# risc0/zeth

Measured on AMD Instinct MI355X. Metric: segments/sec, higher is better.
Workload: dtype u32

## Files before the change

### zeth_amd/build.py

```python
from __future__ import annotations

import hashlib
import os
import subprocess
import sys
from concurrent.futures import ThreadPoolExecutor

HERE = os.path.dirname(os.path.abspath(__file__))
CSRC = os.path.join(HERE, "csrc")
ROOT = os.path.dirname(HERE)
VARIANT = os.environ.get("ZKH_BUILD_VARIANT", "")
LIB = os.path.join(ROOT, ".variants", f"libzkhal_{VARIANT}.so") if VARIANT else os.path.join(HERE, "libzkhal_mi355x.so")
OBJ_DIR = os.path.join(ROOT, ".variants", f"_obj_{VARIANT}") if VARIANT else os.path.join(HERE, "csrc", "_obj")
SOURCES = ["hal.hip", "ntt.hip", "hash.hip", "poly.hip", "circuit.hip", "prover.hip", "verifier.hip", "session.hip", "recursion.hip", "topology.hip", "preflight.hip", "rec_builder.hip", "arguments.hip", "accumulate.hip", "multiplicities.hip", "sort.hip", "columns.hip", "links.hip", "image.hip", "check_rows.hip", "bus.hip"]
HIPCC = os.environ.get("HIPCC", "/opt/rocm/bin/hipcc")
FLAGS = ["--offload-arch=gfx950", "-O3", "-std=c++17", "-fPIC", "-Wno-comment", "-Wno-unused-result"] + os.environ.get("ZKH_BUILD_FLAGS", "").split()
EXTRA_FLAGS = {"hash.hip": ["-mllvm", "-enable-misched=0"], "accumulate.hip": ["-mllvm", "-pragma-unroll-threshold=200000"]}


def _extra(src: str) -> list:
    if src.startswith("eval_check_gen"):
        from .circuits import codegen
        return EXTRA_FLAGS.get(src, []) + codegen.KERNEL_FLAGS
    return EXTRA_FLAGS.get(src, [])


def _deps_digest(src: str) -> str:
    h = hashlib.sha256()
    files = [os.path.join(CSRC, src)]
    files += sorted(os.path.join(CSRC, f) for f in os.listdir(CSRC) if f.endswith(".h"))
    files += [os.path.join(ROOT, "include", f) for f in sorted(os.listdir(os.path.join(ROOT, "include")))]
    for f in files:
        with open(f, "rb") as fh:
            h.update(fh.read())
    h.update(" ".join(FLAGS + _extra(src)).encode())
    return h.hexdigest()


def _compile(src: str, force: bool) -> str:
    obj = os.path.join(OBJ_DIR, src.replace(".hip", ".o"))
    stamp = obj + ".sha"
    digest = _deps_digest(src)
    if not force and os.path.exists(obj) and os.path.exists(stamp) and open(stamp).read() == digest:
        return obj
    if src.startswith("eval_check_gen"):
        from .circuits import bounds
        with open(os.path.join(CSRC, src)) as fh:
            violations, _ = bounds.check_source(fh.read(), src)
        if violations:
            raise RuntimeError(f"{src}: the generated kernels are NOT within bounds (circuits/codegen.py's lazy-arithmetic accounting is wrong); "
                               f"not compiled:\n" + "\n".join(violations[:5]))
    cmd = [HIPCC, *FLAGS, *_extra(src), "-c", os.path.join(CSRC, src), "-o", obj]
    r = subprocess.run(cmd, capture_output=True, text=True)
    if r.returncode != 0:
        raise RuntimeError(f"hipcc failed for {src}:\n{r.stderr[-4000:]}")
    with open(stamp, "w") as fh:
        fh.write(digest)
    return obj


def generate_eval_check() -> list:
    from .circuits import codegen
    return codegen.write_generated(CSRC)


def generate_circuit_descs() -> str:
    import numpy as np
    from .circuits import codegen
    lines = ["// GENERATED by zeth_amd/build.py generate_circuit_descs — do not edit.  The shipped circuit descriptions (circuits/*.py) as data.",
             "#include <cstddef>", "#include <cstdint>", '#include "common.h"', ""]
    names = []
    for name, desc in codegen.shipped().items():
        d = np.asarray(desc, dtype=np.uint32)
        names.append((name, d.size))
        lines.append(f"static const uint32_t desc_{name}[{d.size}] = {{")
        for i in range(0, d.size, 16):
            lines.append("    " + ", ".join(f"0x{int(w):x}" for w in d[i:i + 16]) + ",")
        lines.append("};")
    lines += ["", "namespace {", "struct Shipped { const char* name; const uint32_t* words; size_t n; };", "const Shipped k_shipped[] = {"]
    lines += [f'    {{"{n}", desc_{n}, {sz}}},' for n, sz in names]
    lines += ["};", "}  // namespace", "",
              'extern "C" size_t zkh_shipped_circuit_count() { return sizeof(k_shipped) / sizeof(k_shipped[0]); }',
              'extern "C" const char* zkh_shipped_circuit_name(size_t i) { return i < zkh_shipped_circuit_count() ? k_shipped[i].name : nullptr; }',
              'extern "C" const char* zkh_shipped_circuit_desc(const char* name, const uint32_t** words, size_t* n_words) {',
              '    ZKH_REQUIRE(name && words && n_words, "shipped_circuit_desc: null argument");',
              "    for (const Shipped& s : k_shipped)",
              "        if (strcmp(s.name, name) == 0) { *words = s.words; *n_words = s.n; return nullptr; }",
              '    return zkh::make_err("shipped_circuit_desc: no circuit named %s is built into this library", name);',
              "}", ""]
    src = "\n".join(lines)
    path = os.path.join(CSRC, "circuit_descs_gen.hip")
    try:
        with open(path) as fh:
            if fh.read() == src:
                return "circuit_descs_gen.hip"
    except FileNotFoundError:
        pass
    with open(path, "w") as fh:
        fh.write(src)
    return "circuit_descs_gen.hip"


def build_examples() -> str:
    outs = []
    for name in ("seal_segments", "prove_session", "verify_receipts"):
        src = os.path.join(ROOT, "examples", name + ".cpp")
        out = os.path.join(ROOT, "examples", name)
        outs.append(out)
        deps = [src, os.path.join(ROOT, "include", "zkhal.h"), LIB]
        if os.path.exists(out) and all(os.path.getmtime(out) >= os.path.getmtime(d) for d in deps):
            continue
        cmd = ["g++", "-O2", "-std=c++17", "-Wall", "-I", os.path.join(ROOT, "include"), src, "-o", out, "-L", HERE,
               "-lzkhal_mi355x", "-Wl,-rpath,$ORIGIN/../zeth_amd", "-Wl,-rpath-link,/opt/rocm/lib", "-lpthread"]
        r = subprocess.run(cmd, capture_output=True, text=True)
        if r.returncode != 0:
            raise RuntimeError(f"g++ failed for examples/{name}.cpp:\n{r.stderr[-4000:]}")
    return outs[0]


def build_oracle() -> None:
    subprocess.check_call(["make", "-s", "-C", os.path.join(ROOT, "oracle")])


def build(force: bool = False, verbose: bool = False) -> str:
    os.makedirs(OBJ_DIR, exist_ok=True)
    sources = SOURCES + generate_eval_check() + [generate_circuit_descs()]
    wanted = {s.replace(".hip", ".o") for s in sources}
    for f in os.listdir(OBJ_DIR):
        if f.startswith("eval_check_gen") and f.endswith(".o") and f not in wanted:
            os.remove(os.path.join(OBJ_DIR, f))
    with ThreadPoolExecutor(max_workers=min(os.cpu_count() or 4, len(sources))) as ex:
        objs = list(ex.map(lambda s: _compile(s, force), sources))
    newest = max(os.path.getmtime(o) for o in objs)
    if force or not os.path.exists(LIB) or os.path.getmtime(LIB) < newest:
        cmd = [HIPCC, "--offload-arch=gfx950", "-shared", "-fPIC", *objs, "-o", LIB]
        r = subprocess.run(cmd, capture_output=True, text=True)
        if r.returncode != 0:
            raise RuntimeError(f"link failed:\n{r.stderr[-4000:]}")
    if not VARIANT:
        build_examples()
    if verbose:
        print("built", LIB)
    return LIB


def ensure_built(oracle: bool = False, verbose: bool = False) -> str:
    import fcntl
    stamp = os.path.join(OBJ_DIR, ".tree.sha")
    oracle_built = lambda: any(f.endswith(".so") for f in os.listdir(os.path.join(ROOT, "oracle")))
    try:
        with open(stamp) as fh:
            if os.path.exists(LIB) and fh.read() == _tree_digest() and (not oracle or os.environ.get("ZKH_NO_ORACLE_BUILD") or oracle_built()):
                return LIB
    except OSError:
        pass
    os.makedirs(OBJ_DIR, exist_ok=True)
    with open(os.path.join(OBJ_DIR, ".lock"), "w") as lock:
        fcntl.flock(lock, fcntl.LOCK_EX)
        try:
            digest = _tree_digest()
            current = os.path.exists(LIB) and os.path.exists(stamp) and open(stamp).read() == digest
            if not current:
                build(verbose=verbose)
                with open(stamp, "w") as fh:
                    fh.write(digest)
            if oracle and not os.environ.get("ZKH_NO_ORACLE_BUILD") and not (current and oracle_built()):
                build_oracle()
        finally:
            fcntl.flock(lock, fcntl.LOCK_UN)
    return LIB


def record_tree() -> None:
    os.makedirs(OBJ_DIR, exist_ok=True)
    stamp = os.path.join(OBJ_DIR, ".tree.sha")
    with open(stamp + ".tmp", "w") as fh:
        fh.write(_tree_digest())
    os.replace(stamp + ".tmp", stamp)


def _tree_digest() -> str:
    h = hashlib.sha256()
    files = [os.path.join(CSRC, f) for f in sorted(os.listdir(CSRC))
             if (f.endswith(".hip") or f.endswith(".h")) and not f.startswith("eval_check_gen") and f != "circuit_descs_gen.hip"]
    files += [os.path.join(ROOT, "include", f) for f in sorted(os.listdir(os.path.join(ROOT, "include")))]
    files += [os.path.join(HERE, "circuits", f) for f in sorted(os.listdir(os.path.join(HERE, "circuits"))) if f.endswith((".py", ".json"))]
    files += [os.path.abspath(__file__)] + [os.path.join(ROOT, "examples", f) for f in sorted(os.listdir(os.path.join(ROOT, "examples"))) if f.endswith(".cpp")]
    files += [os.path.join(ROOT, "oracle", f) for f in sorted(os.listdir(os.path.join(ROOT, "oracle"))) if f.endswith((".c", ".h")) or f == "Makefile"]
    for f in files:
        with open(f, "rb") as fh:
            h.update(f.encode() + b"\0" + fh.read())
    h.update(" ".join(FLAGS).encode())
# ... 7 lines not shown
```

### zeth_amd/csrc/common.h

```cpp
#pragma once
#include <hip/hip_runtime.h>

#include <atomic>
#include <cstdarg>
#include <cstdio>
#include <cstdlib>
#include <cstring>
#include <map>
#include <string>
#include <vector>

#include "../../include/zkhal.h"
#include "fp.h"
#include "noise.h"

namespace zkh {

inline const char* make_err(const char* fmt, ...) {
    char buf[512];
    va_list ap;
    va_start(ap, fmt);
    vsnprintf(buf, sizeof buf, fmt, ap);
    va_end(ap);
    return strdup(buf);
}
#define ZKH_HIP(expr)                                                                               \
    do {                                                                                            \
        hipError_t _e = (expr);                                                                     \
        if (_e != hipSuccess) return zkh::make_err("%s failed: %s (%s:%d)", #expr, hipGetErrorString(_e), __FILE__, __LINE__); \
    } while (0)
#define ZKH_TRY(expr)                    \
    do {                                 \
        const char* _err = (expr);       \
        if (_err) return _err;           \
    } while (0)
#define ZKH_REQUIRE(cond, ...)                         \
    do {                                               \
        if (!(cond)) return zkh::make_err(__VA_ARGS__); \
    } while (0)

constexpr int ZKH_P2_PTAB = 486;
constexpr int TW_BITS = 12;
constexpr int TW_SIZE = 1 << TW_BITS;
constexpr int TW_HI_BITS = 14;
constexpr int TW_HI_SIZE = 1 << TW_HI_BITS;
constexpr int MAX_LOG_N = TW_BITS + TW_HI_BITS;
constexpr int LDS_TW_LOG = 12;

struct DeviceTables {
    uint32_t* rc;
    uint32_t* diag;
    uint32_t* tw_fwd_lo; uint32_t* tw_fwd_hi;
    uint32_t* tw_rev_lo; uint32_t* tw_rev_hi;
    uint32_t* tile_fwd;  uint32_t* tile_rev;
    uint32_t* layer_fwd; uint32_t* layer_rev;
    uint32_t* layer_fwd_lazy;
    uint32_t* shift_lo;  uint32_t* shift_hi;
};

struct ProfAgg { uint64_t calls = 0; double ms = 0; double bytes = 0; };
struct ProfPending { std::string name; hipEvent_t a, b; double bytes; };

}

struct zkh_alloc_t {
    void* ptr;
    size_t bytes;
    std::atomic<int> refs;
    bool owned;
    zkh_ctx* ctx;
    zkh_alloc_t(void* p, size_t b, int r, bool o, zkh_ctx* c) : ptr(p), bytes(b), refs(r), owned(o), ctx(c) {}
};

struct zkh_buf {
    zkh_alloc_t* a;
    size_t off, len;
    std::atomic<int> refs;
    zkh_buf(zkh_alloc_t* al, size_t o, size_t l, int r) : a(al), off(o), len(l), refs(r) {}
    uint32_t* ptr() const { return (uint32_t*)a->ptr + off; }
};

struct zkh_ctx {
    int device;
    hipStream_t stream;
    zkh::DeviceTables tab;
    uint32_t rou_fwd[28], rou_rev[28];
    uint32_t h_rc[24 * 29], h_diag[zkh::ZKH_P2_PTAB];
    std::multimap<size_t, void*> pool;
    size_t pool_bytes = 0, live_bytes = 0, peak_bytes = 0;
    bool prof = false;
    std::vector<zkh::ProfPending> pending;
    std::map<std::string, zkh::ProfAgg> agg;
    std::vector<hipEvent_t> event_pool;
    uint32_t* pinned = nullptr;
    size_t pinned_words = 0;
    size_t stage_next = 0, stage_used = 0;
    uint32_t* d_fail = nullptr;
    uint32_t* h_fail = nullptr;
    bool fail_armed = false;
    std::map<void*, size_t> host_blocks;
    size_t h2d_bytes = 0;
};

namespace zkh {

const char* pool_alloc(zkh_ctx* c, size_t bytes, void** out);
void pool_free(zkh_ctx* c, void* p, size_t bytes);
const char* new_buf(zkh_ctx* c, size_t n_words, bool zero, zkh_buf** out);
void prof_begin(zkh_ctx* c, const char* name, double bytes);
void prof_end(zkh_ctx* c);
// ... 38 lines not shown
```

### zeth_amd/csrc/hal.hip

```cpp
#include <algorithm>

#include "common.h"

#include <sys/random.h>
#include "poseidon2.h"
#include "ntt_lazy.h"
#include "../../include/zkh_poseidon2_consts.h"

using namespace zkh;

extern "C" void zkh_free_error(const char* e) { free((void*)e); }
#if ZKH_P2_CONSTS_ARE_PLACEHOLDER
extern "C" const char* zkh_version(void) { return "zkhal-mi355x 0.2.0 (gfx950; poseidon2_consts=placeholder)"; }
#elif ZKH_P2_CONSTS_ARE_DERIVED
extern "C" const char* zkh_version(void) { return "zkhal-mi355x 0.2.0 (gfx950; poseidon2_consts=derived)"; }
#else
extern "C" const char* zkh_version(void) { return "zkhal-mi355x 0.2.0 (gfx950; poseidon2_consts=upstream)"; }
#endif

namespace zkh {

const char* pool_alloc(zkh_ctx* c, size_t bytes, void** out) {
    bytes = (bytes + 255) & ~(size_t)255;
    if (bytes == 0) bytes = 256;
// ... 147 lines not shown
        c->rou_rev[k] = fp_inv(w).v;
    }
    Fp wf = Fp::raw(c->rou_fwd[MAX_LOG_N]), wr = Fp::raw(c->rou_rev[MAX_LOG_N]);
    ZKH_TRY(upload(&c->tab.tw_fwd_lo, powers(wf, TW_SIZE)));
    ZKH_TRY(upload(&c->tab.tw_fwd_hi, powers(fp_pow(wf, TW_SIZE), TW_HI_SIZE)));
    ZKH_TRY(upload(&c->tab.tw_rev_lo, powers(wr, TW_SIZE)));
    ZKH_TRY(upload(&c->tab.tw_rev_hi, powers(fp_pow(wr, TW_SIZE), TW_HI_SIZE)));
    ZKH_TRY(upload(&c->tab.tile_fwd, powers(Fp::raw(c->rou_fwd[LDS_TW_LOG]), 1 << (LDS_TW_LOG - 1))));
    ZKH_TRY(upload(&c->tab.tile_rev, powers(Fp::raw(c->rou_rev[LDS_TW_LOG]), 1 << (LDS_TW_LOG - 1))));
    {
        std::vector<uint32_t> lf(1 << LDS_TW_LOG, R1), lr(1 << LDS_TW_LOG, R1);
        for (int j = 1; j <= LDS_TW_LOG; j++) {
            auto pf = powers(Fp::raw(c->rou_fwd[j]), (size_t)1 << (j - 1)), pr = powers(Fp::raw(c->rou_rev[j]), (size_t)1 << (j - 1));
            for (size_t e = 0; e < pf.size(); e++) { lf[((size_t)1 << (j - 1)) + e] = pf[e]; lr[((size_t)1 << (j - 1)) + e] = pr[e]; }
        }
        ZKH_TRY(upload(&c->tab.layer_fwd, lf));
        ZKH_TRY(upload(&c->tab.layer_rev, lr));
        static_assert(LAZY_TAB_LOG == LDS_TW_LOG, "the lazy table covers the per-layer tables");
        std::vector<uint32_t> lz(LAZY_TAB_WORDS);
        lazy_layer_table(lz.data(), lf.data());
        ZKH_TRY(upload(&c->tab.layer_fwd_lazy, lz));
    }
    Fp three = fp_encode(3);
    ZKH_TRY(upload(&c->tab.shift_lo, powers(three, TW_SIZE)));
    ZKH_TRY(upload(&c->tab.shift_hi, powers(fp_pow(three, TW_SIZE), TW_HI_SIZE)));
    ZKH_TRY(upload(&c->tab.rc, std::vector<uint32_t>(24 * 29)));
    ZKH_TRY(upload(&c->tab.diag, std::vector<uint32_t>(ZKH_P2_PTAB)));
    ZKH_TRY(zkh_poseidon2_set_constants(c, ZKH_P2_ROUND_CONSTANTS, ZKH_P2_M_INT_DIAG));
    ZKH_TRY(ntt_device_init(c));
    ZKH_HIP(hipMalloc((void**)&c->d_fail, 8));
    ZKH_HIP(hipMemsetAsync(c->d_fail, 0, 8, c->stream));
    ZKH_HIP(hipHostMalloc((void**)&c->h_fail, 8, hipHostMallocDefault));
    c->h_fail[0] = c->h_fail[1] = 0;
    return nullptr;
}
extern "C" const char* zkh_ctx_trim(zkh_ctx* c) {
    bind_thread(c);
    ZKH_HIP(hipStreamSynchronize(c->stream));
    for (auto& kv : c->pool) (void)hipFree(kv.second);
    c->pool.clear(); c->pool_bytes = 0;
    return nullptr;
}
extern "C" void zkh_ctx_memory(const zkh_ctx* c, size_t* live, size_t* cached, size_t* peak) {
    if (live) *live = c->live_bytes;
    if (cached) *cached = c->pool_bytes;
    if (peak) *peak = c->peak_bytes;
}
extern "C" void zkh_ctx_destroy(zkh_ctx* c) {
    if (!c) return;
    (void)hipSetDevice(c->device);
    (void)hipStreamSynchronize(c->stream);
    for (auto& kv : c->pool) (void)hipFree(kv.second);
    uint32_t* t[] = {c->tab.rc, c->tab.diag, c->tab.tw_fwd_lo, c->tab.tw_fwd_hi, c->tab.tw_rev_lo, c->tab.tw_rev_hi,
                     c->tab.tile_fwd, c->tab.tile_rev, c->tab.shift_lo, c->tab.shift_hi, c->tab.layer_fwd, c->tab.layer_rev, c->tab.layer_fwd_lazy};
    for (auto p : t) (void)hipFree(p);
    for (auto& p : c->pending) { (void)hipEventDestroy(p.a); (void)hipEventDestroy(p.b); }
    for (auto ev : c->event_pool) (void)hipEventDestroy(ev);
    if (c->pinned) (void)hipHostFree(c->pinned);
    if (c->d_fail) (void)hipFree(c->d_fail);
    if (c->h_fail) (void)hipHostFree(c->h_fail);
    for (auto& kv : c->host_blocks) (void)hipHostFree(kv.first);
    (void)hipStreamDestroy(c->stream);
    delete c;
}
static const char* check_device_fail(zkh_ctx* c) {
    if (!c->fail_armed) return nullptr;
    c->fail_armed = false;
    const uint32_t code = c->h_fail[0], detail = c->h_fail[1];
    if (!code) return nullptr;
    (void)hipMemsetAsync(c->d_fail, 0, 8, c->stream);
    switch (code) {
    case 1: return make_err("combos_prepare_regs: register %u has size 0 or more than `cycles` words (found on the device; the call's combos are unchanged)", detail);
    case 2: return make_err("combos_prepare_regs: register %u names a combo beyond combo_count (found on the device; the call's combos are unchanged)", detail);
    case 3: return make_err("combos_prepare_regs: the register sizes add up to %u U coefficients (+ %d of the check polynomial), more than coeff_u holds (found on the device; the call's combos are unchanged)", detail, ZKH_CHECK_SIZE);
    default: return make_err("a kernel reported failure code %u (%u)", code, detail);
    }
}
static const char* sync_checked(zkh_ctx* c) {
    if (c->fail_armed) ZKH_HIP(hipMemcpyAsync(c->h_fail, c->d_fail, 8, hipMemcpyDeviceToHost, c->stream));
    ZKH_HIP(hipStreamSynchronize(c->stream));
    c->stage_used = 0;
    return check_device_fail(c);
}
extern "C" const char* zkh_sync(zkh_ctx* c) {
    bind_thread(c);
    return sync_checked(c);
}
extern "C" void* zkh_ctx_stream(zkh_ctx* c) { return (void*)c->stream; }

extern "C" const char* zkh_alloc(zkh_ctx* c, const char*, size_t n, int zero, zkh_buf** out) {
    return new_buf(c, n, zero != 0, out);
}
namespace zkh {
constexpr size_t STAGE_SLOT_WORDS = 16384, STAGE_SLOTS = 64;
const char* h2d(zkh_ctx* c, uint32_t* dst, const uint32_t* host, size_t n) {
    if (!n) return nullptr;
    bind_thread(c);
    c->h2d_bytes += n * 4;
    if (n <= STAGE_SLOT_WORDS) {
        ZKH_TRY(ensure_pinned(c, STAGE_SLOT_WORDS * STAGE_SLOTS));
        if (c->stage_used == STAGE_SLOTS) ZKH_TRY(sync_checked(c));
        uint32_t* slot = c->pinned + (size_t)c->stage_next * STAGE_SLOT_WORDS;
        memcpy(slot, host, n * 4);
        ZKH_HIP(hipMemcpyAsync(dst, slot, n * 4, hipMemcpyHostToDevice, c->stream));
        c->stage_next = (c->stage_next + 1) % STAGE_SLOTS;
        c->stage_used++;
        return nullptr;
// ... 388 lines not shown
```

### zeth_amd/csrc/ntt.hip

```cpp
#include "common.h"
#include "ntt_lazy.h"

using namespace zkh;

namespace {

constexpr int NTT_THREADS = 256;

struct PassParams {
    const uint32_t* in;
    uint32_t* out;
    size_t in_col_stride;
    size_t out_col_stride;
    uint32_t log_n;
    uint32_t L, R;
    uint32_t log_t;
    uint32_t expand_bits;
    uint32_t first_layer;
    uint32_t twiddle;
    uint32_t scale;
    uint32_t zk_shift;
    const uint32_t* tile_tw;
    const uint32_t* layer_tw;
    const uint32_t* tw_lo;
    const uint32_t* tw_hi;
    const uint32_t* sh_lo;
    const uint32_t* sh_hi;
    uint32_t tiles_per_col;
    uint32_t lazy;
    uint32_t lazy_comp;
    uint32_t shift16[16];
};

template <bool INVERSE>
__global__ __launch_bounds__(NTT_THREADS) void k_ntt_pass(PassParams p) {
    extern __shared__ __attribute__((aligned(16))) uint32_t tile[];
    const uint32_t T = 1u << p.log_t, rows = 1u << p.R, elems = rows << p.log_t;
    const uint32_t tid = threadIdx.x;
    const uint32_t tile_id = xcd_remap(blockIdx.x, p.tiles_per_col);
    const uint32_t col = blockIdx.y;
    const uint32_t ltiles = 1u << (p.L - p.log_t);
    const uint32_t a = tile_id >> (p.L - p.log_t), lt = tile_id & (ltiles - 1);
    const size_t base = ((size_t)a << (p.L + p.R)) + ((size_t)lt << p.log_t);
    const uint32_t l0 = lt << p.log_t;
    const uint32_t* in = p.in + (size_t)col * p.in_col_stride;
    uint32_t* out = p.out + (size_t)col * p.out_col_stride;
    const uint32_t tw_shift = MAX_LOG_N - (p.L + p.R);
    const uint32_t pad_mask = INVERSE ? 0u : (1u << p.expand_bits) - (1u << (p.first_layer - 1));

    for (uint32_t e = tid; e < elems; e += NTT_THREADS) {
        const uint32_t m = e >> p.log_t, t = e & (T - 1);
        const size_t gi = base + ((size_t)m << p.L) + t;
        uint32_t v = (gi & pad_mask) ? 0u : in[gi >> p.expand_bits];
        if (!INVERSE && p.twiddle) {
            const uint32_t r = __brev(m) >> (32 - p.R);
            const uint32_t ex = ((l0 + t) * r) << tw_shift;
            const uint32_t w = mul_mod(p.tw_lo[ex & (TW_SIZE - 1)], p.tw_hi[ex >> TW_BITS]);
            v = mul_mod(v, w);
        }
        tile[e] = v;
    }
    __syncthreads();

    const uint32_t half_elems = elems >> 1;
    if (INVERSE) {
        for (uint32_t j = p.R; j >= 1; j--) {
            const uint32_t hb = j - 1;
            for (uint32_t q = tid; q < half_elems; q += NTT_THREADS) {
                const uint32_t t = q & (T - 1), mm = q >> p.log_t;
                const uint32_t low = mm & ((1u << hb) - 1), m = ((mm >> hb) << j) | low;
                const uint32_t i0 = (m << p.log_t) | t, i1 = i0 + (1u << (hb + p.log_t));
                const uint32_t x = tile[i0], y = tile[i1];
                const uint32_t w = p.tile_tw[low << (LDS_TW_LOG - j)];
                tile[i0] = add_mod(x, y);
                tile[i1] = mul_mod(x - y + P, w);
            }
            __syncthreads();
        }
    } else {
        for (uint32_t j = p.first_layer; j <= p.R; j++) {
            const uint32_t hb = j - 1;
            for (uint32_t q = tid; q < half_elems; q += NTT_THREADS) {
                const uint32_t t = q & (T - 1), mm = q >> p.log_t;
                const uint32_t low = mm & ((1u << hb) - 1), m = ((mm >> hb) << j) | low;
// ... 358 lines not shown
                }
                radix_layers<2, false, true, 1, LAZY>(u, ltab, 0, 0);
#pragma unroll
                for (int k = 0; k < 4; k++) lds[(m0 + k) * TW + t] = u[k];
            }
            __syncthreads();
#pragma unroll
            for (int k = 0; k < 16; k++) v[k] = lds[(hi * 64 + k * 4 + low) * TW + t];
            radix_layers<4, false, false, 3, LAZY>(v, ltab, low, 0);
#pragma unroll
            for (int k = 0; k < 16; k++) lds[(hi * 64 + k * 4 + low) * TW + t] = v[k];
            __syncthreads();
#pragma unroll
            for (int k = 0; k < 16; k++) v[k] = lds[(k * 64 + g) * TW + t];
            radix_layers<4, false, false, 7, LAZY>(v, ltab, g, 0);
#pragma unroll
            for (int k = 0; k < 16; k++) TILE_OUT(k * 64 + g) = LAZY ? canon((int32_t)v[k]) : v[k];
        }
    } else {
        if (INVERSE) {
#pragma unroll
            for (int k = 0; k < 16; k++) v[k] = TILE_IN(k * 16 + g);
            radix_layers<4, true, false, 5>(v, ltab, g, 0);
#pragma unroll
            for (int k = 0; k < 16; k++) lds[(k * 16 + g) * TW + t] = v[k];
            __syncthreads();
#pragma unroll
            for (int k = 0; k < 16; k++) v[k] = lds[(g * 16 + k) * TW + t];
            radix_layers<4, true, true, 1>(v, ltab, 0, 0);
#pragma unroll
            for (int k = 0; k < 16; k++) {
                uint32_t x = mul_mod(v[k], tw[k]);
                if (p.scale) x = mul_mod(x, p.scale);
                TILE_OUT(g * 16 + k) = x;
            }
        } else {
#pragma unroll
            for (int k = 0; k < 16; k++) {
                const uint32_t x = TILE_IN(g * 16 + k);
                v[k] = LAZY ? (uint32_t)smont((int32_t)x, (int32_t)tw[k]) : mul_mod(x, tw[k]);
            }
            radix_layers<4, false, true, 1, LAZY>(v, ltab, 0, 0);
#pragma unroll
            for (int k = 0; k < 16; k++) lds[(g * 16 + k) * TW + t] = v[k];
            __syncthreads();
#pragma unroll
            for (int k = 0; k < 16; k++) v[k] = lds[(k * 16 + g) * TW + t];
            radix_layers<4, false, false, 5, LAZY>(v, ltab, g, 0);
#pragma unroll
            for (int k = 0; k < 16; k++) TILE_OUT(k * 16 + g) = LAZY ? canon((int32_t)v[k]) : v[k];
        }
    }
}
#undef TILE_IN
#undef TILE_OUT

struct Pass { uint32_t L, R; };
std::vector<Pass> plan_passes(uint32_t log_n) {
    std::vector<Pass> v;
    if (log_n <= 12) { v.push_back({0, log_n}); return v; }
    if (log_n < 18) {
        const uint32_t low = (log_n + 1) / 2;
        v.push_back({0, low});
        v.push_back({low, log_n - low});
        return v;
    }
    const uint32_t rem = log_n - 12;
    v.push_back({0, 12});
    if (rem == 8 || rem == 10 || rem <= 7) v.push_back({12, rem});
    else if (rem == 9) { v.push_back({12, 8}); v.push_back({20, 1}); }
    else if (rem == 11 || rem == 12) { v.push_back({12, 8}); v.push_back({20, rem - 8}); }
    else { v.push_back({12, 10}); v.push_back({22, rem - 10}); }
    return v;
}

const char* run_transform(zkh_ctx* c, bool inverse, const uint32_t* in, size_t in_col_stride, uint32_t* out,
                          size_t out_col_stride, uint32_t log_n, size_t count, uint32_t expand_bits, bool zk, const char* name) {
    ZKH_REQUIRE(log_n <= (uint32_t)MAX_LOG_N, "%s: transform size 2^%u exceeds the supported 2^%d", name, log_n, MAX_LOG_N);
    ZKH_REQUIRE(count <= 65535, "%s: too many columns (%zu)", name, count);
    std::vector<Pass> passes = plan_passes(log_n);
    const size_t n = (size_t)1 << log_n;
    Fp ninv = fp_inv(fp_encode((uint32_t)(n % P)));
    const size_t npass = passes.size();
    const bool lazy = !inverse && npass == 2 && passes[0].R == 12 && (passes[1].R == 8 || passes[1].R == 10) && expand_bits <= 4;
    const uint32_t lazy_reds = lazy ? lazy_reductions(4, expand_bits) + 2 * lazy_reductions(4, 0) + lazy_reductions(passes[1].R, 0) : 0;
    const uint32_t lazy_comp = lazy ? fp_pow(Fp::raw(R2), lazy_reds).v : 0;
    for (size_t pi = 0; pi < npass; pi++) {
        const Pass ps = inverse ? passes[npass - 1 - pi] : passes[pi];
        PassParams p{};
        const bool first = pi == 0, last = pi + 1 == npass;
        p.in = first ? in : out;
        p.in_col_stride = first ? in_col_stride : out_col_stride;
        p.out = out; p.out_col_stride = out_col_stride;
        p.log_n = log_n; p.L = ps.L; p.R = ps.R;
        const bool reg_high = ps.L >= 4 && (ps.R == 8 || ps.R == 10);
        p.log_t = ps.L == 0 ? 0 : (ps.L < 4 ? ps.L : 4);
        if (ps.L != 0 && !reg_high && ps.R < 12) p.log_t = std::max<uint32_t>(p.log_t, std::min<uint32_t>(ps.L, 12 - ps.R));
        while (p.R + p.log_t > 14 && p.log_t > 0) p.log_t--;
        p.expand_bits = (!inverse && first) ? expand_bits : 0;
        p.first_layer = (!inverse && first) ? std::min(expand_bits, ps.R) + 1 : 1;
        p.twiddle = ps.L != 0;
        p.scale = (inverse && last) ? ninv.v : 0;
        p.zk_shift = (inverse && last && zk) ? 1 : 0;
        p.lazy = lazy; p.lazy_comp = lazy_comp;
        p.tile_tw = inverse ? c->tab.tile_rev : c->tab.tile_fwd;
        p.layer_tw = inverse ? c->tab.layer_rev : (lazy ? c->tab.layer_fwd_lazy : c->tab.layer_fwd);
        p.tw_lo = inverse ? c->tab.tw_rev_lo : c->tab.tw_fwd_lo;
        p.tw_hi = inverse ? c->tab.tw_rev_hi : c->tab.tw_fwd_hi;
        p.sh_lo = c->tab.shift_lo; p.sh_hi = c->tab.shift_hi;
        if (p.zk_shift && log_n >= 4) {
            const Fp three = fp_encode(3);
            for (uint32_t k = 0; k < 16; k++)
                p.shift16[k] = (ninv * fp_pow(three, (uint64_t)(bitrev32(k) >> 28) << (log_n - 4))).v;
        }
        p.tiles_per_col = (uint32_t)(n >> (p.R + p.log_t));
        const size_t lds = ((size_t)4 << (p.R + p.log_t));
        dim3 grid(p.tiles_per_col, (unsigned)count);
        const double alg_bytes = pi == 0 ? 4.0 * count * (double)(((size_t)1 << log_n) >> expand_bits) + 4.0 * count * (double)n : 0.0;
        const bool scale_here = p.scale != 0;
        const bool k_low = ps.L == 0 && ps.R == 12 && p.expand_bits <= 4;
        const bool k_h10 = !k_low && ps.L >= 4 && p.log_t == 4 && ps.R == 10 && !(scale_here && p.zk_shift);
        const bool k_h8 = !k_low && !k_h10 && ps.L >= 4 && p.log_t == 4 && ps.R == 8 && !(scale_here && p.zk_shift);
        const bool k_top = !k_low && !k_h10 && !k_h8 && ps.L >= 12 && ps.L + ps.R == log_n && ps.R >= 1 && ps.R <= 4 && p.twiddle &&
                           p.expand_bits == 0 && p.first_layer == 1 && !scale_here && !p.zk_shift;
        const std::string pname = std::string(name) + (k_low ? ":k_ntt_low12" : k_h10 ? ":k_ntt_high10" : k_h8 ? ":k_ntt_high8" : k_top ? ":k_ntt_top" : ":k_ntt_pass");
        ProfScope prof(c, pname.c_str(), alg_bytes);
        if (ps.L == 0 && ps.R == 12 && p.expand_bits <= 4) {
            if (inverse) k_ntt_low12<true><<<grid, 256, 0, c->stream>>>(p);
            else if (lazy) k_ntt_low12<false, true><<<grid, 256, 0, c->stream>>>(p);
            else k_ntt_low12<false><<<grid, 256, 0, c->stream>>>(p);
        } else if (ps.L >= 4 && p.log_t == 4 && ps.R == 10 && !(scale_here && p.zk_shift)) {
            if (inverse) k_ntt_high<10, true><<<grid, 1024, lds, c->stream>>>(p);
            else if (lazy) k_ntt_high<10, false, true><<<grid, 1024, lds, c->stream>>>(p);
            else k_ntt_high<10, false><<<grid, 1024, lds, c->stream>>>(p);
        } else if (ps.L >= 4 && p.log_t == 4 && ps.R == 8 && !(scale_here && p.zk_shift)) {
            if (inverse) k_ntt_high<8, true><<<grid, 256, lds, c->stream>>>(p);
            else if (lazy) k_ntt_high<8, false, true><<<grid, 256, lds, c->stream>>>(p);
            else k_ntt_high<8, false><<<grid, 256, lds, c->stream>>>(p);
        } else if (k_top) {
            const dim3 tg((unsigned)(((size_t)1 << ps.L) >> 10), (unsigned)count);
            switch (ps.R * 2 + (inverse ? 1 : 0)) {
            case 2: k_ntt_top<1, false><<<tg, 256, 0, c->stream>>>(p); break;
            case 3: k_ntt_top<1, true><<<tg, 256, 0, c->stream>>>(p); break;
            case 4: k_ntt_top<2, false><<<tg, 256, 0, c->stream>>>(p); break;
            case 5: k_ntt_top<2, true><<<tg, 256, 0, c->stream>>>(p); break;
            case 6: k_ntt_top<3, false><<<tg, 256, 0, c->stream>>>(p); break;
            case 7: k_ntt_top<3, true><<<tg, 256, 0, c->stream>>>(p); break;
            case 8: k_ntt_top<4, false><<<tg, 256, 0, c->stream>>>(p); break;
            default: k_ntt_top<4, true><<<tg, 256, 0, c->stream>>>(p); break;
            }
        } else if (inverse) k_ntt_pass<true><<<grid, NTT_THREADS, lds, c->stream>>>(p);
        else k_ntt_pass<false><<<grid, NTT_THREADS, lds, c->stream>>>(p);
        ZKH_TRY(last_launch_error(name));
    }
    return nullptr;
}

}

const char* zkh::ntt_device_init(zkh_ctx* c) {
    bind_thread(c);
    ZKH_HIP(hipFuncSetAttribute((const void*)k_ntt_high<10, true>, hipFuncAttributeMaxDynamicSharedMemorySize, 65536));
    ZKH_HIP(hipFuncSetAttribute((const void*)k_ntt_high<10, false>, hipFuncAttributeMaxDynamicSharedMemorySize, 65536));
    ZKH_HIP(hipFuncSetAttribute((const void*)k_ntt_high<10, false, true>, hipFuncAttributeMaxDynamicSharedMemorySize, 65536));
    return nullptr;
}

static const char* interpolate_impl(zkh_ctx* c, zkh_buf* io, size_t count, bool zk, const char* name) {
    ZKH_REQUIRE(count && io->len % count == 0, "%s: size %zu not a multiple of count %zu", name, io->len, count);
    const size_t n = io->len / count;
    const uint32_t log_n = log2_ceil(n);
    ZKH_REQUIRE(((size_t)1 << log_n) == n, "%s: column length %zu is not a power of two", name, n);
    return run_transform(c, true, io->ptr(), n, io->ptr(), n, log_n, count, 0, zk, name);
}
extern "C" const char* zkh_batch_interpolate_ntt(zkh_ctx* c, zkh_buf* io, size_t count) {
    return interpolate_impl(c, io, count, false, "batch_interpolate_ntt");
}
extern "C" const char* zkh_batch_interpolate_ntt_zk_shift(zkh_ctx* c, zkh_buf* io, size_t count) {
    return interpolate_impl(c, io, count, true, "batch_interpolate_ntt_zk_shift");
}
extern "C" const char* zkh_batch_interpolate_ntt_from(zkh_ctx* c, zkh_buf* out, const zkh_buf* in, size_t count, int zk_shift) {
    ZKH_REQUIRE(count && in->len % count == 0 && out->len == in->len, "batch_interpolate_ntt_from: shape mismatch");
    const size_t n = in->len / count;
    const uint32_t log_n = log2_ceil(n);
    ZKH_REQUIRE(((size_t)1 << log_n) == n, "batch_interpolate_ntt_from: column length %zu is not a power of two", n);
    return run_transform(c, true, in->ptr(), n, out->ptr(), n, log_n, count, 0, zk_shift != 0, "batch_interpolate_ntt_from");
}
extern "C" const char* zkh_batch_expand_into_evaluate_ntt(zkh_ctx* c, zkh_buf* out, const zkh_buf* in, size_t count,
                                                          size_t expand_bits) {
    ZKH_REQUIRE(count && out->len % count == 0 && in->len % count == 0, "batch_expand_into_evaluate_ntt: sizes not multiples of count");
    const size_t n_out = out->len / count, n_in = in->len / count;
    const uint32_t log_n = log2_ceil(n_out);
    ZKH_REQUIRE(((size_t)1 << log_n) == n_out, "batch_expand_into_evaluate_ntt: column length %zu is not a power of two", n_out);
    ZKH_REQUIRE(expand_bits <= log_n, "batch_expand_into_evaluate_ntt: expand_bits %zu too large for columns of %zu", expand_bits, n_out);
    ZKH_REQUIRE((n_in << expand_bits) == n_out, "batch_expand_into_evaluate_ntt: out column %zu != in column %zu << %zu", n_out, n_in, expand_bits);
    return run_transform(c, false, in->ptr(), n_in, out->ptr(), n_out, log_n, count, (uint32_t)expand_bits, false,
                         "batch_expand_into_evaluate_ntt");
}
extern "C" const char* zkh_zk_shift(zkh_ctx* c, zkh_buf* io, size_t count) {
    ZKH_REQUIRE(count && io->len % count == 0, "zk_shift: size not a multiple of count");
    const size_t n = io->len / count;
    const uint32_t log_n = log2_ceil(n);
    ZKH_REQUIRE(((size_t)1 << log_n) == n && log_n <= (uint32_t)MAX_LOG_N, "zk_shift: bad column length %zu", n);
    ProfScope prof(c, "zk_shift", 8.0 * io->len);
    k_zk_shift<<<(unsigned)((io->len + 255) / 256), 256, 0, c->stream>>>(io->ptr(), io->len, log_n, c->tab.shift_lo, c->tab.shift_hi);
    return last_launch_error("zk_shift");
}
extern "C" const char* zkh_batch_bit_reverse(zkh_ctx* c, zkh_buf* io, size_t count) {
    ZKH_REQUIRE(count && io->len % count == 0, "batch_bit_reverse: size not a multiple of count");
    const size_t n = io->len / count;
    const uint32_t log_n = log2_ceil(n);
    ZKH_REQUIRE(((size_t)1 << log_n) == n, "batch_bit_reverse: column length %zu is not a power of two", n);
    ProfScope prof(c, "batch_bit_reverse", 8.0 * io->len);
    if (log_n >= 2 * BR_H + 1 && count <= 65535) {
        dim3 grid(1u << (log_n - 2 * BR_H), (unsigned)count);
        k_bit_reverse_tiled<<<grid, 256, 0, c->stream>>>(io->ptr(), log_n, n);
    } else {
// ... 5 lines not shown
```

### zeth_amd/csrc/ntt_lazy.h

```cpp
#pragma once
#include "fp.h"

#ifndef ZKH_LAZY_SUM
#define ZKH_LAZY_SUM(t) ((void)0)
#endif

namespace zkh {

constexpr int LAZY_TAB_LOG = 12;
constexpr uint32_t LAZY_TAB_MONT = 1u << LAZY_TAB_LOG;
constexpr uint32_t LAZY_TAB_WORDS = 2u << LAZY_TAB_LOG;

inline void lazy_layer_table(uint32_t* out, const uint32_t* layer_fwd) {
    for (uint32_t i = 0; i < LAZY_TAB_MONT; i++) {
        out[i] = (uint32_t)center(mont_reduce((uint64_t)layer_fwd[i]));
        out[LAZY_TAB_MONT + i] = (uint32_t)center(layer_fwd[i]);
    }
}

template <bool UNIFORM>
ZKH_HD int64_t lazy_mad(int32_t a, int32_t w, int64_t acc) {
    if constexpr (UNIFORM) return mad_i64_k(a, w, acc);
    else return mad_i64(a, w, acc);
}
// ... 15 lines not shown
    const int32_t nwa = -wa, nwb0 = -wb0, nwb1 = -wb1;
    const int64_t x0 = (int64_t)(int32_t)v0, x2 = (int64_t)(int32_t)v2;
    const int32_t x1 = (int32_t)v1, x3 = (int32_t)v3;
    const int32_t u2 = lazy_reduce(lazy_mad<UNIFORM>(x3, wa, x2));
    const int32_t u3 = lazy_reduce(lazy_mad<UNIFORM>(x3, nwa, x2));
    const int64_t sp = lazy_mad<UNIFORM>(x1, wa, x0), sm = lazy_mad<UNIFORM>(x1, nwa, x0);
    v0 = (uint32_t)lazy_reduce(lazy_mad<UNIFORM>(u2, wb0, sp));
    v2 = (uint32_t)lazy_reduce(lazy_mad<UNIFORM>(u2, nwb0, sp));
    v1 = (uint32_t)lazy_reduce(lazy_mad<UNIFORM>(u3, wb1, sm));
    v3 = (uint32_t)lazy_reduce(lazy_mad<UNIFORM>(u3, nwb1, sm));
}

ZKH_HD uint32_t lazy_reductions(uint32_t logr, uint32_t first_b) {
    const uint32_t live = first_b < logr ? logr - first_b : 0;
    return (live + 1) / 2;
}

template <int LOGR, bool BASE0, int J_LO>
ZKH_HD void lazy_layers(uint32_t (&v)[1 << LOGR], const uint32_t* __restrict__ ltab, const uint32_t base_low, const int first_b) {
    static_assert(LOGR % 2 == 0, "lazy rounds hold an even number of layers");
    constexpr int N = 1 << LOGR;
#pragma unroll
    for (int b = 0; b < LOGR; b += 2) {
        const uint32_t* twa = ltab + (1u << (J_LO + b - 1));
        const uint32_t* twb = ltab + LAZY_TAB_MONT + (1u << (J_LO + b));
        if (b >= first_b) {
#pragma unroll
            for (int kk = 0; kk < (1 << b); kk++) {
                const uint32_t e = base_low + ((uint32_t)kk << (J_LO - 1));
                const int32_t wa = (BASE0 && kk == 0) ? 1 : (int32_t)twa[e];
                const int32_t wb0 = (BASE0 && kk == 0) ? (int32_t)R1 : (int32_t)twb[e];
                const int32_t wb1 = (int32_t)twb[e + ((1u << b) << (J_LO - 1))];
#pragma unroll
                for (int hi = 0; hi < (N >> (b + 2)); hi++) {
                    const int k = (hi << (b + 2)) | kk;
                    lazy_pair<BASE0>(v[k], v[k + (1 << b)], v[k + (2 << b)], v[k + (3 << b)], wa, wb0, wb1);
                }
            }
        } else if (b + 1 >= first_b) {
            const uint32_t* tw1 = ltab + (1u << (J_LO + b));
#pragma unroll
            for (int kk = 0; kk < (2 << b); kk++) {
                const int32_t w = (BASE0 && kk == 0) ? 1 : (int32_t)tw1[base_low + ((uint32_t)kk << (J_LO - 1))];
#pragma unroll
                for (int hi = 0; hi < (N >> (b + 2)); hi++) {
                    const int k = (hi << (b + 2)) | kk;
                    lazy_single<BASE0>(v[k], v[k + (2 << b)], w);
                }
            }
        }
    }
}

}
```

Before: 44.55.

## Add lazy-reduction block inverse NTT kernels with precomputed per-layer twiddle table

Adds new inverse NTT kernels (k_intt_low12, k_intt_high<8/10>) that apply two layers at a time using lazy signed Montgomery reductions and a precomputed bit-reversed per-layer twiddle table of 2^22 entries. The accumulated Montgomery factors are folded into the final scale and zk-shift constants. The goal is fewer reductions and fewer twiddle computations in the inverse transform. In exchange it adds a 32 MB device table built lazily on the host, and the build now also produces a separate DIF library variant with these kernels turned off.

```diff
diff --git a/zeth_amd/build.py b/zeth_amd/build.py
--- a/zeth_amd/build.py
+++ b/zeth_amd/build.py
@@ -16,6 +16,8 @@
 HIPCC = os.environ.get("HIPCC", "/opt/rocm/bin/hipcc")
 FLAGS = ["--offload-arch=gfx950", "-O3", "-std=c++17", "-fPIC", "-Wno-comment", "-Wno-unused-result"] + os.environ.get("ZKH_BUILD_FLAGS", "").split()
 EXTRA_FLAGS = {"hash.hip": ["-mllvm", "-enable-misched=0"], "accumulate.hip": ["-mllvm", "-pragma-unroll-threshold=200000"]}
+DIF_LIB = os.path.join(HERE, "libzkhal_mi355x_dif.so")
+DIF_FLAGS = ["-DZKH_NTT_INVERSE_DIF"]
 
 
 def _extra(src: str) -> list:
@@ -37,10 +39,10 @@
     return h.hexdigest()
 
 
-def _compile(src: str, force: bool) -> str:
-    obj = os.path.join(OBJ_DIR, src.replace(".hip", ".o"))
+def _compile(src: str, force: bool, more: tuple = (), tag: str = "") -> str:
+    obj = os.path.join(OBJ_DIR, src.replace(".hip", tag + ".o"))
     stamp = obj + ".sha"
-    digest = _deps_digest(src)
+    digest = _deps_digest(src) + " ".join(more)
     if not force and os.path.exists(obj) and os.path.exists(stamp) and open(stamp).read() == digest:
         return obj
     if src.startswith("eval_check_gen"):
@@ -50,7 +52,7 @@
         if violations:
             raise RuntimeError(f"{src}: the generated kernels are NOT within bounds (circuits/codegen.py's lazy-arithmetic accounting is wrong); "
                                f"not compiled:\n" + "\n".join(violations[:5]))
-    cmd = [HIPCC, *FLAGS, *_extra(src), "-c", os.path.join(CSRC, src), "-o", obj]
+    cmd = [HIPCC, *FLAGS, *_extra(src), *more, "-c", os.path.join(CSRC, src), "-o", obj]
     r = subprocess.run(cmd, capture_output=True, text=True)
     if r.returncode != 0:
         raise RuntimeError(f"hipcc failed for {src}:\n{r.stderr[-4000:]}")
@@ -130,7 +132,9 @@
         if f.startswith("eval_check_gen") and f.endswith(".o") and f not in wanted:
             os.remove(os.path.join(OBJ_DIR, f))
     with ThreadPoolExecutor(max_workers=min(os.cpu_count() or 4, len(sources))) as ex:
+        dif = ex.submit(_compile, "ntt.hip", force, tuple(DIF_FLAGS), "_dif") if not VARIANT else None
         objs = list(ex.map(lambda s: _compile(s, force), sources))
+        dif_obj = dif.result() if dif else None
     newest = max(os.path.getmtime(o) for o in objs)
     if force or not os.path.exists(LIB) or os.path.getmtime(LIB) < newest:
         cmd = [HIPCC, "--offload-arch=gfx950", "-shared", "-fPIC", *objs, "-o", LIB]
@@ -138,6 +142,12 @@
         if r.returncode != 0:
             raise RuntimeError(f"link failed:\n{r.stderr[-4000:]}")
     if not VARIANT:
+        ntt_obj = os.path.join(OBJ_DIR, "ntt.o")
+        dif_objs = [dif_obj if o == ntt_obj else o for o in objs]
+        if force or not os.path.exists(DIF_LIB) or os.path.getmtime(DIF_LIB) < max(os.path.getmtime(o) for o in dif_objs):
+            r = subprocess.run([HIPCC, "--offload-arch=gfx950", "-shared", "-fPIC", *dif_objs, "-o", DIF_LIB], capture_output=True, text=True)
+            if r.returncode != 0:
+                raise RuntimeError(f"link failed:\n{r.stderr[-4000:]}")
         build_examples()
     if verbose:
         print("built", LIB)
diff --git a/zeth_amd/csrc/common.h b/zeth_amd/csrc/common.h
--- a/zeth_amd/csrc/common.h
+++ b/zeth_amd/csrc/common.h
@@ -56,6 +56,7 @@
     uint32_t* layer_fwd; uint32_t* layer_rev;
     uint32_t* layer_fwd_lazy;
     uint32_t* shift_lo;  uint32_t* shift_hi;
+    uint32_t* block_rev;
 };
 
 struct ProfAgg { uint64_t calls = 0; double ms = 0; double bytes = 0; };
diff --git a/zeth_amd/csrc/hal.hip b/zeth_amd/csrc/hal.hip
--- a/zeth_amd/csrc/hal.hip
+++ b/zeth_amd/csrc/hal.hip
@@ -223,7 +223,7 @@
     (void)hipStreamSynchronize(c->stream);
     for (auto& kv : c->pool) (void)hipFree(kv.second);
     uint32_t* t[] = {c->tab.rc, c->tab.diag, c->tab.tw_fwd_lo, c->tab.tw_fwd_hi, c->tab.tw_rev_lo, c->tab.tw_rev_hi,
-                     c->tab.tile_fwd, c->tab.tile_rev, c->tab.shift_lo, c->tab.shift_hi, c->tab.layer_fwd, c->tab.layer_rev, c->tab.layer_fwd_lazy};
+                     c->tab.tile_fwd, c->tab.tile_rev, c->tab.shift_lo, c->tab.shift_hi, c->tab.layer_fwd, c->tab.layer_rev, c->tab.layer_fwd_lazy, c->tab.block_rev};
     for (auto p : t) (void)hipFree(p);
     for (auto& p : c->pending) { (void)hipEventDestroy(p.a); (void)hipEventDestroy(p.b); }
     for (auto ev : c->event_pool) (void)hipEventDestroy(ev);
diff --git a/zeth_amd/csrc/ntt.hip b/zeth_amd/csrc/ntt.hip
--- a/zeth_amd/csrc/ntt.hip
+++ b/zeth_amd/csrc/ntt.hip
@@ -30,6 +30,7 @@
     uint32_t lazy;
     uint32_t lazy_comp;
     uint32_t shift16[16];
+    const uint32_t* block_tw;
 };
 
 template <bool INVERSE>
@@ -494,6 +495,141 @@
         }
     }
 }
+
+template <int LOGR>
+__device__ __forceinline__ void block_twiddles(int32_t (&w)[1 << LOGR], const uint32_t* __restrict__ T, const uint32_t s0, const uint32_t prefix) {
+#pragma unroll
+    for (int s = 0; s < LOGR; s++) {
+        const uint32_t* src = T + ((s & 1) ? BLOCK_TAB_MONT : 0u) + ((1u << (s0 + s)) + (prefix << s));
+        if (s == 0) w[1] = (int32_t)src[0];
+        else if (s == 1) { const uint2 q = *(const uint2*)src; w[2] = (int32_t)q.x; w[3] = (int32_t)q.y; }
+        else {
+#pragma unroll
+            for (int i = 0; i < (1 << s); i += 4) {
+                const uint4 q = *(const uint4*)(src + i);
+                w[(1 << s) + i] = (int32_t)q.x; w[(1 << s) + i + 1] = (int32_t)q.y; w[(1 << s) + i + 2] = (int32_t)q.z; w[(1 << s) + i + 3] = (int32_t)q.w;
+            }
+        }
+    }
+}
+template <int LOGR>
+__device__ __forceinline__ void block_twiddles_top(int32_t (&w)[1 << LOGR], const uint32_t* __restrict__ T) {
+#pragma unroll
+    for (int e = 1; e < (1 << LOGR); e++) {
+        const int s = 31 - __builtin_clz((unsigned)e);
+        w[e] = e == 1 ? 1 : e == 2 ? (int32_t)R1 : (int32_t)T[((s & 1) ? BLOCK_TAB_MONT : 0u) + e];
+    }
+}
+#define BLOCK_TW(w) [&](int s, int i) -> int32_t { return (w)[(1 << s) + i]; }
+
+template <int RH>
+__global__ __launch_bounds__(1 << RH) void k_intt_high(PassParams p) {
+    constexpr int LT = 4;
+    constexpr uint32_t TW = 1u << LT;
+    extern __shared__ __attribute__((aligned(16))) uint32_t lds[];
+    const uint32_t tid = threadIdx.x, t = tid & (TW - 1), g = tid >> LT;
+    const uint32_t tile_id = xcd_remap(blockIdx.x, p.tiles_per_col), col = blockIdx.y;
+    const uint32_t lt_bits = p.L - LT;
+    const uint32_t a = tile_id >> lt_bits, lt = tile_id & ((1u << lt_bits) - 1);
+    const size_t base = ((size_t)a << (p.L + RH)) + ((size_t)lt << LT);
+    const char* in = (const char*)(p.in + (size_t)col * p.in_col_stride + base);
+    char* out = (char*)(p.out + (size_t)col * p.out_col_stride + base);
+    const uint32_t tb = t * 4u;
+    const uint32_t* __restrict__ T = p.block_tw;
+    uint32_t v[16];
+    int32_t w[16];
+    if (RH == 10) {
+        const uint32_t hi = g >> 2, low = g & 3;
+#pragma unroll
+        for (int k = 0; k < 16; k++) v[k] = TILE_IN(k * 64 + g);
+        block_twiddles_top<4>(w, T);
+        lazy_block_layers<4, true>(v, BLOCK_TW(w));
+#pragma unroll
+        for (int k = 0; k < 16; k++) lds[(k * 64 + g) * TW + t] = v[k];
+        __syncthreads();
+#pragma unroll
+        for (int k = 0; k < 16; k++) v[k] = lds[(hi * 64 + k * 4 + low) * TW + t];
+        block_twiddles<4>(w, T, 4, hi);
+        lazy_block_layers<4, false>(v, BLOCK_TW(w));
+#pragma unroll
+        for (int k = 0; k < 16; k++) lds[(hi * 64 + k * 4 + low) * TW + t] = v[k];
+        __syncthreads();
+#pragma unroll
+        for (int i = 0; i < 4; i++) {
+            uint32_t u[4];
+            int32_t w2[4];
+            const uint32_t m0 = (g * 4 + i) * 4;
+#pragma unroll
+            for (int k = 0; k < 4; k++) u[k] = lds[(m0 + k) * TW + t];
+            block_twiddles<2>(w2, T, 8, g * 4 + i);
+            lazy_block_layers<2, false>(u, BLOCK_TW(w2));
+#pragma unroll
+            for (int k = 0; k < 4; k++) TILE_OUT(m0 + k) = u[k];
+        }
+    } else {
+#pragma unroll
+        for (int k = 0; k < 16; k++) v[k] = TILE_IN(k * 16 + g);
+        block_twiddles_top<4>(w, T);
+        lazy_block_layers<4, true>(v, BLOCK_TW(w));
+#pragma unroll
+        for (int k = 0; k < 16; k++) lds[(k * 16 + g) * TW + t] = v[k];
+        __syncthreads();
+#pragma unroll
+        for (int k = 0; k < 16; k++) v[k] = lds[(g * 16 + k) * TW + t];
+        block_twiddles<4>(w, T, 4, g);
+        lazy_block_layers<4, false>(v, BLOCK_TW(w));
+#pragma unroll
+        for (int k = 0; k < 16; k++) TILE_OUT(g * 16 + k) = v[k];
+    }
+}
+
+__global__ __launch_bounds__(256) void k_intt_low12(PassParams p) {
+    __shared__ __attribute__((aligned(16))) uint32_t lds[4096];
+    const uint32_t tid = threadIdx.x;
+    const uint32_t tile = xcd_remap(blockIdx.x, p.tiles_per_col), col = blockIdx.y;
+    const size_t base = (size_t)tile << 12;
+    const uint32_t* in = p.in + (size_t)col * p.in_col_stride;
+    uint32_t* out = p.out + (size_t)col * p.out_col_stride;
+    const uint32_t* __restrict__ T = p.block_tw;
+    const uint32_t rh = p.log_n - 12;
+    const uint32_t hi = tid >> 4, low = tid & 15;
+    uint32_t v[16];
+    int32_t w[16];
+#pragma unroll
+    for (int k = 0; k < 16; k++) v[k] = in[base + k * 256 + tid];
+    block_twiddles<4>(w, T, rh, tile);
+    lazy_block_layers<4, true>(v, BLOCK_TW(w));
+#pragma unroll
+    for (int k = 0; k < 16; k++) lds[k * 256 + tid] = v[k];
+    __syncthreads();
+#pragma unroll
+    for (int k = 0; k < 16; k++) v[k] = lds[hi * 256 + k * 16 + low];
+    block_twiddles<4>(w, T, rh + 4, (tile << 4) | hi);
+    lazy_block_layers<4, false>(v, BLOCK_TW(w));
+#pragma unroll
+    for (int k = 0; k < 16; k++) lds[hi * 256 + k * 16 + low] = v[k];
+    __syncthreads();
+#pragma unroll
+    for (int q = 0; q < 4; q++) {
+        const uint4 x = ((const uint4*)lds)[tid * 4 + q];
+        v[4 * q] = x.x; v[4 * q + 1] = x.y; v[4 * q + 2] = x.z; v[4 * q + 3] = x.w;
+    }
+    block_twiddles<4>(w, T, rh + 8, (tile << 8) | tid);
+    lazy_block_layers<4, false>(v, BLOCK_TW(w));
+    const size_t pos0 = base + (size_t)tid * 16;
+    if (p.zk_shift) {
+        const uint32_t ex = __brev((uint32_t)pos0) >> (32 - p.log_n);
+        const int32_t b = (int32_t)mul_mod(p.sh_lo[ex & (TW_SIZE - 1)], p.sh_hi[ex >> TW_BITS]);
+#pragma unroll
+        for (int k = 0; k < 16; k++) v[k] = canon(lazy_scale<true>(lazy_scale<false>((int32_t)v[k], b), (int32_t)p.shift16[k]));
+    } else {
+#pragma unroll
+        for (int k = 0; k < 16; k++) v[k] = canon(lazy_scale<true>((int32_t)v[k], (int32_t)p.scale));
+    }
+#pragma unroll
+    for (int q = 0; q < 4; q++) ((uint4*)(out + pos0))[q] = make_uint4(v[4 * q], v[4 * q + 1], v[4 * q + 2], v[4 * q + 3]);
+}
+#undef BLOCK_TW
 #undef TILE_IN
 #undef TILE_OUT
 
@@ -514,6 +650,22 @@
     else if (rem == 11 || rem == 12) { v.push_back({12, 8}); v.push_back({20, rem - 8}); }
     else { v.push_back({12, 10}); v.push_back({22, rem - 10}); }
     return v;
+}
+
+const char* block_table(zkh_ctx* c, const uint32_t** out) {
+    if (!c->tab.block_rev) {
+        std::vector<uint32_t> t(BLOCK_TAB_WORDS);
+        block_twiddle_table(t.data(), c->rou_rev);
+        uint32_t* d = nullptr;
+        ZKH_HIP(hipMalloc((void**)&d, t.size() * 4));
+        if (hipError_t e = hipMemcpy(d, t.data(), t.size() * 4, hipMemcpyHostToDevice); e != hipSuccess) {
+            (void)hipFree(d);
+            return make_err("hipMemcpy of the block-twiddle table failed: %s", hipGetErrorString(e));
+        }
+        c->tab.block_rev = d;
+    }
+    *out = c->tab.block_rev;
+    return nullptr;
 }
 
 const char* run_transform(zkh_ctx* c, bool inverse, const uint32_t* in, size_t in_col_stride, uint32_t* out,
@@ -527,6 +679,19 @@
     const bool lazy = !inverse && npass == 2 && passes[0].R == 12 && (passes[1].R == 8 || passes[1].R == 10) && expand_bits <= 4;
     const uint32_t lazy_reds = lazy ? lazy_reductions(4, expand_bits) + 2 * lazy_reductions(4, 0) + lazy_reductions(passes[1].R, 0) : 0;
     const uint32_t lazy_comp = lazy ? fp_pow(Fp::raw(R2), lazy_reds).v : 0;
+#if defined(ZKH_NTT_INVERSE_DIF)
+    const bool block = false;
+#else
+    const bool block = inverse && npass == 2 && passes[0].L == 0 && passes[0].R == 12 && passes[1].L == 12 && (passes[1].R == 8 || passes[1].R == 10) &&
+                       log_n <= (uint32_t)BLOCK_TAB_LOG;
+#endif
+    const uint32_t* block_tw = nullptr;
+    Fp block_scale = ninv;
+    if (block) {
+        bind_thread(c);
+        ZKH_TRY(block_table(c, &block_tw));
+        block_scale = ninv * fp_pow(Fp::raw(R2), passes[1].R / 2 + 6);
+    }
     for (size_t pi = 0; pi < npass; pi++) {
         const Pass ps = inverse ? passes[npass - 1 - pi] : passes[pi];
         PassParams p{};
@@ -542,7 +707,8 @@
         p.expand_bits = (!inverse && first) ? expand_bits : 0;
         p.first_layer = (!inverse && first) ? std::min(expand_bits, ps.R) + 1 : 1;
         p.twiddle = ps.L != 0;
-        p.scale = (inverse && last) ? ninv.v : 0;
+        p.scale = (inverse && last) ? (block ? (uint32_t)center(block_scale.v) : ninv.v) : 0;
+        p.block_tw = block_tw;
         p.zk_shift = (inverse && last && zk) ? 1 : 0;
         p.lazy = lazy; p.lazy_comp = lazy_comp;
         p.tile_tw = inverse ? c->tab.tile_rev : c->tab.tile_fwd;
@@ -553,7 +719,8 @@
         if (p.zk_shift && log_n >= 4) {
             const Fp three = fp_encode(3);
             for (uint32_t k = 0; k < 16; k++)
-                p.shift16[k] = (ninv * fp_pow(three, (uint64_t)(bitrev32(k) >> 28) << (log_n - 4))).v;
+                p.shift16[k] = (block_scale * fp_pow(three, (uint64_t)(bitrev32(k) >> 28) << (log_n - 4))).v;
+            if (block) for (uint32_t k = 0; k < 16; k++) p.shift16[k] = (uint32_t)center(p.shift16[k]);
         }
         p.tiles_per_col = (uint32_t)(n >> (p.R + p.log_t));
         const size_t lds = ((size_t)4 << (p.R + p.log_t));
@@ -568,15 +735,18 @@
         const std::string pname = std::string(name) + (k_low ? ":k_ntt_low12" : k_h10 ? ":k_ntt_high10" : k_h8 ? ":k_ntt_high8" : k_top ? ":k_ntt_top" : ":k_ntt_pass");
         ProfScope prof(c, pname.c_str(), alg_bytes);
         if (ps.L == 0 && ps.R == 12 && p.expand_bits <= 4) {
-            if (inverse) k_ntt_low12<true><<<grid, 256, 0, c->stream>>>(p);
+            if (block) k_intt_low12<<<grid, 256, 0, c->stream>>>(p);
+            else if (inverse) k_ntt_low12<true><<<grid, 256, 0, c->stream>>>(p);
             else if (lazy) k_ntt_low12<false, true><<<grid, 256, 0, c->stream>>>(p);
             else k_ntt_low12<false><<<grid, 256, 0, c->stream>>>(p);
         } else if (ps.L >= 4 && p.log_t == 4 && ps.R == 10 && !(scale_here && p.zk_shift)) {
-            if (inverse) k_ntt_high<10, true><<<grid, 1024, lds, c->stream>>>(p);
+            if (block) k_intt_high<10><<<grid, 1024, lds, c->stream>>>(p);
+            else if (inverse) k_ntt_high<10, true><<<grid, 1024, lds, c->stream>>>(p);
             else if (lazy) k_ntt_high<10, false, true><<<grid, 1024, lds, c->stream>>>(p);
             else k_ntt_high<10, false><<<grid, 1024, lds, c->stream>>>(p);
         } else if (ps.L >= 4 && p.log_t == 4 && ps.R == 8 && !(scale_here && p.zk_shift)) {
-            if (inverse) k_ntt_high<8, true><<<grid, 256, lds, c->stream>>>(p);
+            if (block) k_intt_high<8><<<grid, 256, lds, c->stream>>>(p);
+            else if (inverse) k_ntt_high<8, true><<<grid, 256, lds, c->stream>>>(p);
             else if (lazy) k_ntt_high<8, false, true><<<grid, 256, lds, c->stream>>>(p);
             else k_ntt_high<8, false><<<grid, 256, lds, c->stream>>>(p);
         } else if (k_top) {
@@ -605,6 +775,7 @@
     ZKH_HIP(hipFuncSetAttribute((const void*)k_ntt_high<10, true>, hipFuncAttributeMaxDynamicSharedMemorySize, 65536));
     ZKH_HIP(hipFuncSetAttribute((const void*)k_ntt_high<10, false>, hipFuncAttributeMaxDynamicSharedMemorySize, 65536));
     ZKH_HIP(hipFuncSetAttribute((const void*)k_ntt_high<10, false, true>, hipFuncAttributeMaxDynamicSharedMemorySize, 65536));
+    ZKH_HIP(hipFuncSetAttribute((const void*)k_intt_high<10>, hipFuncAttributeMaxDynamicSharedMemorySize, 65536));
     return nullptr;
 }
 
diff --git a/zeth_amd/csrc/ntt_lazy.h b/zeth_amd/csrc/ntt_lazy.h
--- a/zeth_amd/csrc/ntt_lazy.h
+++ b/zeth_amd/csrc/ntt_lazy.h
@@ -91,4 +91,44 @@
     }
 }
 
+constexpr int BLOCK_TAB_LOG = 22;
+constexpr uint32_t BLOCK_TAB_MONT = 1u << BLOCK_TAB_LOG;
+constexpr uint32_t BLOCK_TAB_WORDS = 2u << BLOCK_TAB_LOG;
+
+inline void block_twiddle_table(uint32_t* out, const uint32_t* rou_rev) {
+    out[0] = out[BLOCK_TAB_MONT] = 0;
+    for (int l = 0; l < BLOCK_TAB_LOG; l++) {
+        const uint32_t m = 1u << l;
+        uint32_t w = R1;
+        for (uint32_t e = 0; e < m; e++) {
+            const uint32_t i = l ? bitrev32(e) >> (32 - l) : 0;
+            out[m + i] = (uint32_t)center(mont_reduce((uint64_t)w));
+            out[BLOCK_TAB_MONT + m + i] = (uint32_t)center(w);
+            w = mul_mod(w, rou_rev[l + 1]);
+        }
+    }
 }
+
+template <int LOGR, bool UNIFORM, class TW>
+ZKH_HD void lazy_block_layers(uint32_t (&v)[1 << LOGR], const TW& tw) {
+    static_assert(LOGR % 2 == 0, "lazy rounds hold an even number of layers");
+    constexpr int N = 1 << LOGR;
+#pragma unroll
+    for (int s = 0; s < LOGR; s += 2) {
+        const int D = N >> (s + 1);
+#pragma unroll
+        for (int i = 0; i < (1 << s); i++) {
+            const int32_t wa = tw(s, i), wb0 = tw(s + 1, 2 * i), wb1 = tw(s + 1, 2 * i + 1);
+#pragma unroll
+            for (int j = 0; j < D / 2; j++) {
+                const int k = i * 2 * D + j;
+                lazy_pair<UNIFORM>(v[k], v[k + D], v[k + D / 2], v[k + D / 2 + D], wa, wb0, wb1);
+            }
+        }
+    }
+}
+
+template <bool UNIFORM>
+ZKH_HD int32_t lazy_scale(int32_t v, int32_t c) { return lazy_reduce(lazy_mad<UNIFORM>(v, c, (int64_t)0)); }
+
+}
```

Result: no change. 44.80, median of 2 (+0.6%).
